# marvinpfoertner/linpde-gp

Hardware: AMD Instinct MI355X
Metric: condition+predict fp64 GFLOP/s (algorithmic), N=16384 Poisson-2D (higher is better)
Workload: dtype f64; 1 GPU; poisson2d_dirichlet_128x128; n_collocation=16384, n_other_observations=512, n_total=16896, m_predict=4096, multi_gpu=single GPU, rccl_ranks=0, device=(gfx950:sramecc+:xnack-), lazy_factorization=True, fused_factor_and_predict=True

## Files before the change

### linpde-gp_amd/csrc/api.hip

```cpp

#include <cstdarg>
#include <cstdlib>
#include <cstring>
#include <memory>

#include <rccl/rccl.h>

#include "lpgp_internal.h"

namespace lpgp {

static hipEvent_t get_event(lpgp_ctx* ctx) {
  if (!ctx->event_pool.empty()) {
    hipEvent_t e = ctx->event_pool.back();
    ctx->event_pool.pop_back();
    return e;
  }
  hipEvent_t e = nullptr;
  (void)hipEventCreate(&e);
  return e;
}

void prof_begin(lpgp_ctx* ctx, hipStream_t stream, int kernel, double flops, double bytes) {
  ctx->prof_open = 0;
// ... 255 lines not shown
  mat->cap = cap;
  mat->lr_cap = lr;
  mat->lc_cap = lc;
  mat->has_r = 0;
  return 0;
}

static void scatter_padded(const lpgp_mat* mat, const double* logical, double* padded) {
  std::memset(padded, 0, (size_t)mat->pn * sizeof(double));
  for (const auto& b : mat->blocks) std::memcpy(padded + b.poff, logical + b.off, (size_t)b.n * sizeof(double));
}
static void gather_padded(const lpgp_mat* mat, const double* padded, double* logical) {
  for (const auto& b : mat->blocks) std::memcpy(logical + b.off, padded + b.poff, (size_t)b.n * sizeof(double));
}

}

using namespace lpgp;

extern "C" {

const char* lpgp_last_error(void) { return lpgp::last_error(); }

int lpgp_init(int device, lpgp_ctx** out) {
  LPGP_CHECK(out != nullptr, "lpgp_init: null out");
  int ndev = 0;
  LPGP_HIP(hipGetDeviceCount(&ndev));
  LPGP_CHECK(ndev > 0, "lpgp_init: no HIP device visible (this library has no CPU fallback)");
  LPGP_CHECK(device >= 0 && device < ndev, "lpgp_init: device %d out of range (%d visible)", device, ndev);
  LPGP_HIP(hipSetDevice(device));
  lpgp_ctx* ctx = new lpgp_ctx();
  ctx->device = device;
  options_from_env(*ctx);
  hipDeviceProp_t prop;
  LPGP_HIP(hipGetDeviceProperties(&prop, device));
  ctx->cus = prop.multiProcessorCount;
  int lo = 0, hi = 0;
  LPGP_HIP(hipDeviceGetStreamPriorityRange(&lo, &hi));
  LPGP_HIP(hipStreamCreateWithPriority(&ctx->s_main, hipStreamNonBlocking, hi));
  auto masked_stream = [&](int nreserve, hipStream_t* out) {
    *out = nullptr;
    if (nreserve == 0 || nreserve >= ctx->cus) return;
    const int words = (ctx->cus + 31) / 32;
    std::vector<uint32_t> mask(words, 0u);
    for (int cu = 0; cu < ctx->cus; ++cu) mask[cu / 32] |= (1u << (cu % 32));
    for (int r = 0; r < nreserve; ++r) mask[r / 32] &= ~(1u << (r % 32));
    if (hipExtStreamCreateWithCUMask(out, (uint32_t)words, mask.data()) != hipSuccess) {
      (void)hipGetLastError();
      *out = nullptr;
    }
  };
  if (ctx->single_stream) {
    ctx->s_upd = ctx->s_upd_narrow = ctx->s_upd_all = ctx->s_outer = ctx->s_main;
  } else {
  masked_stream(ctx->reserve_cus, &ctx->s_upd);
  if (!ctx->s_upd) LPGP_HIP(hipStreamCreateWithPriority(&ctx->s_upd, hipStreamNonBlocking, lo));
  masked_stream(ctx->reserve_narrow, &ctx->s_upd_narrow);
  LPGP_HIP(hipStreamCreateWithPriority(&ctx->s_upd_all, hipStreamNonBlocking, lo));
  masked_stream(ctx->reserve_cus, &ctx->s_outer);
  if (!ctx->s_outer) LPGP_HIP(hipStreamCreateWithPriority(&ctx->s_outer, hipStreamNonBlocking, lo));
  }
  for (int i = 0; i < 2; ++i) {
    LPGP_HIP(hipEventCreateWithFlags(&ctx->ev_outer[i], hipEventDisableTiming));
    LPGP_HIP(hipEventCreateWithFlags(&ctx->ev_outer_fact[i], hipEventDisableTiming));
    LPGP_HIP(hipEventCreateWithFlags(&ctx->ev_outer_a1[i], hipEventDisableTiming));
  }
  for (int i = 0; i < 4; ++i) LPGP_HIP(hipEventCreateWithFlags(&ctx->ev_ride[i], hipEventDisableTiming));
  LPGP_HIP(hipEventCreateWithFlags(&ctx->ev_chain_pre, hipEventDisableTiming));
  LPGP_HIP(hipEventCreateWithFlags(&ctx->ev_chain_rows, hipEventDisableTiming));
  LPGP_HIP(hipEventCreateWithFlags(&ctx->ev_append[0], hipEventDisableTiming));
  LPGP_HIP(hipEventCreateWithFlags(&ctx->ev_append[1], hipEventDisableTiming));
  for (int i = 0; i < 2; ++i) {
    LPGP_HIP(hipEventCreateWithFlags(&ctx->ev_panel[i], hipEventDisableTiming));
    LPGP_HIP(hipEventCreateWithFlags(&ctx->ev_upd[i], hipEventDisableTiming));
  }
  for (auto& sl : ctx->desc_ring) {
    LPGP_HIP(hipHostMalloc(&sl.h, sizeof(DevDesc), hipHostMallocDefault));
    LPGP_HIP(hipMalloc(&sl.d, sizeof(DevDesc)));
    LPGP_HIP(hipEventCreateWithFlags(&sl.done, hipEventDisableTiming));
  }
  LPGP_HIP(hipMalloc(&ctx->d_info, sizeof(int)));
  LPGP_HIP(hipHostMalloc(&ctx->h_info_pinned, 64, hipHostMallocDefault));
  *out = ctx;
  return 0;
}

int lpgp_finalize(lpgp_ctx* ctx) {
  if (!ctx) return 0;
  (void)hipSetDevice(ctx->device);
  if (ctx->nccl_comm && ctx->world > 1 && sync_stream(ctx, ctx->s_main) != 0) {
  }
  (void)hipDeviceSynchronize();
  for (auto& p : ctx->pending) {
    (void)hipEventDestroy(p.e0);
    (void)hipEventDestroy(p.e1);
  }
  for (auto e : ctx->event_pool) (void)hipEventDestroy(e);
  for (int i = 0; i < 4; ++i) (void)hipEventDestroy(ctx->ev_ride[i]);
  (void)hipEventDestroy(ctx->ev_chain_pre);
  if (ctx->ev_chain_rows) (void)hipEventDestroy(ctx->ev_chain_rows);
  for (auto& e : ctx->ev_append) if (e) (void)hipEventDestroy(e);
  for (int i = 0; i < 2; ++i) {
    (void)hipEventDestroy(ctx->ev_panel[i]);
    (void)hipEventDestroy(ctx->ev_upd[i]);
    (void)hipEventDestroy(ctx->ev_outer[i]);
    (void)hipEventDestroy(ctx->ev_outer_fact[i]);
    (void)hipEventDestroy(ctx->ev_outer_a1[i]);
  }
  for (auto& sl : ctx->desc_ring) {
    (void)hipHostFree(sl.h);
    (void)hipFree(sl.d);
    (void)hipEventDestroy(sl.done);
  }
  (void)hipFree(ctx->d_info);
  if (ctx->d_chain_flags) (void)hipFree(ctx->d_chain_flags);
  (void)hipHostFree(ctx->h_info_pinned);
  if (ctx->h_stage) (void)hipHostFree(ctx->h_stage);
  for (auto& b : ctx->pts_pool) (void)hipFree(b.p);
  ctx->pts_pool.clear();
  for (auto& sl : ctx->pts_ring) {
    if (sl.h) (void)hipHostFree(sl.h);
    if (sl.done) (void)hipEventDestroy(sl.done);
  }
  if (ctx->h_stage_r) (void)hipHostFree(ctx->h_stage_r);
  if (ctx->ev_stage_r) (void)hipEventDestroy(ctx->ev_stage_r);
  if (ctx->d_tmp) (void)hipFree(ctx->d_tmp);
  for (size_t r = 0; r < ctx->ipc_peer.size(); ++r)
    if ((int)r != ctx->rank && ctx->ipc_peer[r]) (void)hipIpcCloseMemHandle(ctx->ipc_peer[r]);
  if (ctx->ipc_window) (void)hipFree(ctx->ipc_window);
  for (int i = 0; i < 2; ++i)
    if (ctx->ev_ipc[i]) (void)hipEventDestroy(ctx->ev_ipc[i]);
// ... 11 lines not shown
  for (auto& b : ctx->pool) (void)hipFree(b.p);
  ctx->pool.clear();
  if (!ctx->single_stream) {
    (void)hipStreamDestroy(ctx->s_upd);
    if (ctx->s_upd_narrow) (void)hipStreamDestroy(ctx->s_upd_narrow);
    (void)hipStreamDestroy(ctx->s_upd_all);
    if (ctx->s_outer) (void)hipStreamDestroy(ctx->s_outer);
  }
  (void)hipStreamDestroy(ctx->s_main);
  delete ctx;
  return 0;
}

int lpgp_device_info(lpgp_ctx* ctx, char* name, int len, int* cus, int64_t* hbm_bytes) {
  LPGP_DEVICE(ctx);
  hipDeviceProp_t prop;
  LPGP_HIP(hipGetDeviceProperties(&prop, ctx->device));
  if (name && len > 0) {
    std::snprintf(name, (size_t)len, "%s (%s)", prop.name, prop.gcnArchName);
  }
  if (cus) *cus = prop.multiProcessorCount;
  if (hbm_bytes) *hbm_bytes = (int64_t)prop.totalGlobalMem;
  return 0;
}

int lpgp_sync(lpgp_ctx* ctx) {
  LPGP_HIP(hipSetDevice(ctx->device));
  LPGP_HIP(hipDeviceSynchronize());
  return 0;
}

#define ROUTE(name) {"route_" #name, &lpgp_ctx::RouteCounts::name}
static const struct { const char* key; int64_t lpgp_ctx::RouteCounts::*count; } kRoutes[] = {
    ROUTE(ride_done), ROUTE(ride_aug), ROUTE(ride_b2b), ROUTE(ride), ROUTE(ride_vchain), ROUTE(ride_two), ROUTE(ride_outer),
    ROUTE(solve_two_level), ROUTE(solve_ahead), ROUTE(solve_tiles)};
#undef ROUTE
static const struct { const char* key; int64_t lpgp_ctx::*field; } kEvidence[] = {
    {"inverse_diag_panel", &lpgp_ctx::inverse_diag_panel}, {"evidence_h2d_bytes", &lpgp_ctx::evidence_h2d_bytes}, {"evidence_d2h_bytes", &lpgp_ctx::evidence_d2h_bytes}};

int lpgp_get_option(lpgp_ctx* ctx, const char* key, int64_t* value) {
  LPGP_CHECK(ctx && key && value, "lpgp_get_option: null argument");
  const int rc = option_get(*ctx, key, value);
  if (rc == 0) return 0;
  if (std::strcmp(key, "live_mats") == 0) {
    *value = ctx->live_mats;
    return 0;
  }
  for (const auto& r : kRoutes)
    if (std::strcmp(key, r.key) == 0) {
      *value = ctx->route.*r.count;
      return 0;
    }
  for (const auto& r : kEvidence)
    if (std::strcmp(key, r.key) == 0) {
      *value = ctx->*r.field;
      return 0;
    }
  return rc;
}

int lpgp_set_option(lpgp_ctx* ctx, const char* key, int64_t value) {
  LPGP_DEVICE(ctx);
  if (key && std::strcmp(key, kEvidence[0].key) == 0) {
    LPGP_CHECK(value >= TILE && value <= 4096 && value % TILE == 0, "inverse_diag_panel must be a multiple of %d in %d .. 4096", TILE, TILE);
    ctx->inverse_diag_panel = value;
    return 0;
  }
  return option_set(*ctx, key, value);
}

int lpgp_dist_unique_id(char* out128) {
  LPGP_CHECK(out128 != nullptr, "lpgp_dist_unique_id: null argument");
  static_assert(sizeof(ncclUniqueId) == 128, "ncclUniqueId size");
  ncclUniqueId id;
  ncclResult_t r = ncclGetUniqueId(&id);
  LPGP_CHECK(r == ncclSuccess, "ncclGetUniqueId: %s", ncclGetErrorString(r));
  std::memcpy(out128, &id, 128);
  return 0;
}

static void choose_grid(lpgp_ctx* ctx, int world) {
  if (ctx->grid_set && ctx->pr * ctx->pc == world) return;
  ctx->pr = world;
  ctx->pc = 1;
}

static int dist_fail(lpgp_ctx* ctx, int rc);

int lpgp_dist_set_grid(lpgp_ctx* ctx, int32_t pr, int32_t pc) {
  LPGP_CHECK(ctx && pr >= 1 && pc >= 1 && pr <= 8 && pc <= 8, "lpgp_dist_set_grid: bad grid %d x %d", pr, pc);
  if (ctx->distributed()) {
    LPGP_CHECK(pr * pc == ctx->world, "lpgp_dist_set_grid: grid %d x %d does not match %d ranks", pr, pc, ctx->world);
    LPGP_CHECK(ctx->live_mats == 0, "lpgp_dist_set_grid: %d matrices / right-hand sides of the current grid are still alive", ctx->live_mats);
  }
  ctx->pr = pr;
  ctx->pc = pc;
  ctx->grid_set = 1;
  return 0;
// ... 982 lines not shown
  const bool via_z = mean_host && var_host && !mat->has_w && mat->has_r;
  if (mean_host && !via_z) {
    LPGP_CHECK(mat->has_w, "lpgp_predict: representer weights not computed (call lpgp_solve_weights%s)",
               var_host ? " or lpgp_mat_set_residual" : "");
    LPGP_TRY(reduce_read_back(ctx, mat, K, mat->w, false, prior_mean_host, nullptr, mean_host, nullptr, nullptr));
  }
  if (var_host) {
    LPGP_CHECK(kxx_host != nullptr, "lpgp_predict: kxx_host required for the variance");
    double* zcol = K->v + (int64_t)K->m * K->ld;
    if (via_z)
      LPGP_HIP(hipMemcpyAsync(zcol, mat->r(), (size_t)mat->pn * sizeof(double), hipMemcpyDeviceToDevice, ctx->s_main));
    LPGP_TRY(solve_lower(ctx, mat, K->v, K->ld, K->m_pad));
    LPGP_TRY(reduce_read_back(ctx, mat, K, via_z ? zcol : nullptr, true, prior_mean_host, kxx_host, mean_host, var_host, nullptr));
  }
  return 0;
}

int lpgp_potrf_predict(lpgp_ctx* ctx, lpgp_mat* mat, lpgp_rhs* K, const double* prior_mean_host, const double* kxx_host,
                       double* mean_host, double* var_host) {
  LPGP_CHECK(ctx && mat && K && kxx_host && mean_host && var_host, "lpgp_potrf_predict: null argument");
  LPGP_DEVICE(ctx);
  LPGP_MAT_ALIVE(mat, "lpgp_potrf_predict");
  LPGP_CHECK(!ctx->distributed(), "lpgp_potrf_predict: single GPU only (a multi-GPU job factors collectively: lpgp_potrf, lpgp_predict)");
  LPGP_CHECK(mat->hidden.empty(), "lpgp_potrf_predict: a strict prefix of the blocks is in view");
  LPGP_CHECK(K->ld == mat->pn && mat->pn > 0, "lpgp_potrf_predict: right-hand side built for another matrix size");
  LPGP_CHECK(mat->has_r, "lpgp_potrf_predict: no residual resident (lpgp_mat_set_residual)");
  LPGP_TRY(ensure_tmp(ctx, 2 * K->m_pad));
  LPGP_TRY(ensure_stage(ctx, 2 * K->m_pad));
  LPGP_TRY(rhs_clear_unassembled(ctx, mat, K));
  double* zcol = K->v + (int64_t)K->m * K->ld;
  LPGP_HIP(hipMemcpyAsync(zcol, mat->r(), (size_t)mat->pn * sizeof(double), hipMemcpyDeviceToDevice, ctx->s_main));
  const bool fresh = mat->pn_fact < mat->pn;
  ctx->d_info_cur = mat->d_status;
  const int rc = potrf_predict_blocked(ctx, mat, mat->pn_fact / TILE, mat->pn / TILE, K->v, K->ld, K->m_pad);
  if (rc != 0) {
    if (fresh) mat->poisoned = 1;
    return rc;
  }
  if (fresh) {
    mat->pn_fact = mat->pn;
    mat->unchecked = 1;
    mat->has_w = 0;
  }
  mat->status_known = 0;
  int* const hinfo = ctx->h_info_pinned + 4;
  LPGP_TRY(reduce_read_back(ctx, mat, K, zcol, true, prior_mean_host, kxx_host, mean_host, var_host, hinfo));
  if (mat->unchecked) {
    mat->status_value = *hinfo;
    mat->status_known = 1;
  }
  return 0;
}

int lpgp_rhs_inner(lpgp_ctx* ctx, lpgp_rhs* A, lpgp_rhs* B, double* out_host) {
  LPGP_CHECK(ctx && A && B && out_host, "lpgp_rhs_inner: null argument");
  LPGP_DEVICE(ctx);
  LPGP_CHECK(A->ld == B->ld, "lpgp_rhs_inner: row mismatch");
  const int64_t ma = A->m_pad, mb = B->m_pad;
  std::vector<double> h((size_t)ma * mb);
  DevBuf dc;
  LPGP_TRY(DevBuf::raw(h.size() * sizeof(double), &dc));
  StreamDrain drain{ctx->s_main};
  GemmArgs g;
  g.A = A->v; g.B = B->v; g.C = dc.as(); g.lda = A->ld; g.ldb = B->ld; g.ldc = ma;
  g.mt = (int)(ma / TILE); g.nt = (int)(mb / TILE); g.k = (int)A->ld; g.alpha = 1.0; g.beta = 0.0;
  g.tri = 0;
  LPGP_TRY(launch_gemm(ctx, ctx->s_main, 1, 1, g, LPGP_K_GEMM));
// ... 295 lines not shown
```

### linpde-gp_amd/csrc/lpgp_internal.h

```cpp
#pragma once

#include <hip/hip_runtime.h>

#include <cstdint>
#include <cstdio>
#include <string>
#include <vector>

#include "lpgp.h"
#include "lpgp_desc.h"
#include "options.h"

namespace lpgp {

struct Cyc {
  int32_t P = 1, me = 0, nbt = 4;
};
__host__ __device__ inline int cyc_owner(const Cyc& c, int g) { return (g / c.nbt) % c.P; }
__host__ __device__ inline int cyc_before(const Cyc& c, int g) {
  const int B = g / c.nbt, rem = g - B * c.nbt;
  return ((B + c.P - 1 - c.me) / c.P) * c.nbt + ((B % c.P) == c.me ? rem : 0);
}
__host__ __device__ inline int cyc_l2g(const Cyc& c, int l) {
  const int lb = l / c.nbt;
// ... 25 lines not shown
  do {                            \
    int _rc = (expr);             \
    if (_rc != 0) return _rc;     \
  } while (0)
#define LPGP_TRY(expr) LPGP_TRY_RC(expr)

struct ProfSlot {
  double ms = 0.0;
  int64_t launches = 0;
  double flops = 0.0;
  double bytes = 0.0;
};

struct PendingEvent {
  hipEvent_t e0, e1;
  int kernel;
};

}

struct lpgp_ctx : lpgp::Options {
  int device = 0;
  int cus = 0;
  hipStream_t s_main = nullptr;
  hipStream_t s_upd = nullptr;
  hipStream_t s_upd_narrow = nullptr;
  hipStream_t s_upd_all = nullptr;
  hipStream_t s_outer = nullptr;
  hipEvent_t ev_outer[2] = {nullptr, nullptr};
  hipEvent_t ev_outer_fact[2] = {nullptr, nullptr};
  hipEvent_t ev_outer_a1[2] = {nullptr, nullptr};
  hipEvent_t ev_chain_pre = nullptr;
  hipEvent_t ev_ride[4] = {nullptr, nullptr, nullptr, nullptr};
  hipEvent_t ev_append[2] = {nullptr, nullptr};
  hipEvent_t ev_chain_rows = nullptr;
  int* d_chain_flags = nullptr;
  int64_t chain_launches = 0;
  int* chain_last_slot = nullptr;
  int chain_last_p0 = -1;
  struct RouteCounts {
    int64_t ride_done = 0;
    int64_t ride_aug = 0;
    int64_t ride_b2b = 0;
    int64_t ride = 0;
    int64_t ride_vchain = 0;
    int64_t ride_two = 0;
    int64_t ride_outer = 0;
    int64_t solve_two_level = 0;
    int64_t solve_ahead = 0;
    int64_t solve_tiles = 0;
  } route;
  hipEvent_t ev_panel[2] = {nullptr, nullptr};
  hipEvent_t ev_upd[2] = {nullptr, nullptr};
  int64_t inverse_diag_panel = 4096;
  int64_t evidence_h2d_bytes = 0, evidence_d2h_bytes = 0;
  int panel_lds_extra = 0;
  static constexpr int DESC_RING = 8;
  struct DescSlot { lpgp::DevDesc* h = nullptr; lpgp::DevDesc* d = nullptr; hipEvent_t done = nullptr; bool used = false; };
  DescSlot desc_ring[DESC_RING];
  int desc_next = 0;
  int* d_info = nullptr;
  int* d_info_cur = nullptr;
  int* h_info_pinned = nullptr;
  double* d_tmp = nullptr;
  int64_t tmp_cap = 0;
  double* h_stage = nullptr;
  double* h_stage_r = nullptr;
  int64_t stage_r_cap = 0;
  hipEvent_t ev_stage_r = nullptr;
  int64_t stage_cap = 0;
  struct PoolBuf { void* p; size_t bytes; };
  std::vector<PoolBuf> pool;
  std::vector<PoolBuf> pts_pool;
  static constexpr int PTS_SLOTS = 8;
  static constexpr size_t PTS_SLOT_BYTES = 64 << 10;
  struct PtsSlot { void* h = nullptr; hipEvent_t done = nullptr; bool used = false; };
  PtsSlot pts_ring[PTS_SLOTS];
  int pts_next = 0;
  int rank = 0, world = 1;
  int pr = 1, pc = 1;
  int grid_set = 0;
  int dist_broken = 0;
  int live_mats = 0;
  double comm_bytes_sent = 0.0, comm_bytes_recv = 0.0;
  hipStream_t s_comm = nullptr;
  hipEvent_t ev_comm[2] = {nullptr, nullptr};
  void* nccl_comm = nullptr;
  void* nccl_comm_bulk = nullptr;
// ... 196 lines not shown
  int32_t occ3 = 1;
  int32_t sshift = 3;
  int32_t dense = 0;
  int32_t ntiles = 0, chunk = 0, nbands = 0, band = 8;
  static constexpr int MAXB = 192;
  int32_t band_prefix[MAXB + 1];
  int32_t cyc = 0;
  Cyc rowc, colc;
  int32_t rt0 = 0, ct0 = 0, g0 = 0;
  unsigned long long* stamps = nullptr;
  unsigned long long* timeline = nullptr;
};
int launch_gemm(lpgp_ctx* ctx, hipStream_t stream, int ta, int tb, const GemmArgs& g, int prof_kernel);
int stair_enumerate_host(const GemmArgs& g, int32_t* out, int64_t cap);
int64_t gemm_valid_tiles(const GemmArgs& g);
int launch_trsv_tile(lpgp_ctx* ctx, hipStream_t stream, double* V, int64_t ldv, const double* linv, const double* L, int64_t ldl,
                     int nt, int prof_kernel);
int launch_trsm_tile(lpgp_ctx* ctx, hipStream_t stream, double* X, int64_t ldx, const double* linv, const double* L, int64_t ldl,
                     int mt, int prof_kernel);
int launch_trsv_panel(lpgp_ctx* ctx, hipStream_t stream, double* V, int64_t ldv, const double* linv, const double* L, int64_t ldl,
                      int nt_rows, int nt_cols, int prof_kernel);
int launch_trsv_panel_ahead(lpgp_ctx* ctx, hipStream_t stream, double* V, int64_t ldv, const double* linv, const double* L, const double* Lprev,
                            int64_t ldl, int nt_rows, int nt_cols, int prof_kernel);
int launch_trsm_panel(lpgp_ctx* ctx, hipStream_t stream, double* X, int64_t ldx, const double* linv, const double* L, int64_t ldl,
                      int nt_cols, int mt, int prof_kernel);

int launch_panel_chain(lpgp_ctx* ctx, hipStream_t stream, lpgp_mat* mat, int p0, int T, int* d_info, bool rows_here = true, bool ahead = false);
int launch_panel_chain_rows(lpgp_ctx* ctx, hipStream_t stream, lpgp_mat* mat, int p0, int T, int* d_info);
int launch_panel_chain_v(lpgp_ctx* ctx, hipStream_t stream, lpgp_mat* mat, int p0, double* V, int64_t ldv, int64_t cols, int* d_info);
int debug_tile_xcc(int32_t* out8, int reset);
int launch_potrf_tile(lpgp_ctx* ctx, hipStream_t stream, double* a, int64_t lda, double* linv,
                      int* d_info, int info_base);
int potrf_blocked(lpgp_ctx* ctx, lpgp_mat* mat, int64_t t_done, int64_t T, int32_t* info);
int potrf_predict_blocked(lpgp_ctx* ctx, lpgp_mat* mat, int64_t t_done, int64_t T, double* v, int64_t ldv, int64_t m_pad);
int potrf_dist(lpgp_ctx* ctx, lpgp_mat* mat, int64_t t_done, int64_t T, int32_t* info);
int trsm_lower_dist(lpgp_ctx* ctx, lpgp_mat* mat, int64_t T, double* v, int64_t ldv, int64_t m_pad);
int trsm_lower_t_dist(lpgp_ctx* ctx, lpgp_mat* mat, int64_t T, double* v, int64_t ldv, int64_t m_pad);
int factor_to_host_dist(lpgp_ctx* ctx, lpgp_mat* mat, double* out_padded );
int copy2d(hipStream_t st, double* dst, int64_t ldd, const double* src, int64_t lds, int64_t rows, int64_t cols);
int trsm_lower_blocked(lpgp_ctx* ctx, lpgp_mat* mat, int64_t T, double* v, int64_t ldv, int64_t m_pad);
int trsm_lower_t_blocked(lpgp_ctx* ctx, lpgp_mat* mat, int64_t T, double* v, int64_t ldv, int64_t m_pad);
int solve_vec(lpgp_ctx* ctx, lpgp_mat* mat, int64_t T, double* v, double* tmp, int* info);
int solve_vec_resident(lpgp_ctx* ctx, lpgp_mat* mat, int64_t T, double* v, double* tmp, int* info);
int solve_vec_fwd(lpgp_ctx* ctx, hipStream_t st, lpgp_mat* mat, int64_t T, double* b, double* x);
int solve_vec_fwd_resident(lpgp_ctx* ctx, lpgp_mat* mat, int64_t T, const double* b, double* x, int* info);
int mat_evidence(lpgp_ctx* ctx, lpgp_mat* mat, const double* r_host, double out_host[2]);
int mat_inverse_diag(lpgp_ctx* ctx, lpgp_mat* mat, double* out_host);
int mat_loo(lpgp_ctx* ctx, lpgp_mat* mat, const double* r_host, const double* y_host, double* mean_host, double* var_host, double* logp_host);
int mat_inverse_into(lpgp_ctx* ctx, lpgp_mat* mat, lpgp_mat* out);
int mat_evidence_grad(lpgp_ctx* ctx, lpgp_mat* mat, const lpgp_mat* ginv, const lpgp_mat* dG, const double* r_host, double out_host[2]);
int mat_evidence_grad_diag(lpgp_ctx* ctx, lpgp_mat* mat, const lpgp_mat* ginv, int32_t bi, const double* v_host, double scalar, const double* r_host,
                           double out_host[2]);
int factor_matmul(lpgp_ctx* ctx, lpgp_mat* mat, const double* Z_host, int64_t s, const double* shift_host, double* out_host);

int launch_assemble(lpgp_ctx* ctx, hipStream_t stream, const DevDesc& host_desc, const double* x0,
                    int64_t n0, int64_t n0_pad, const double* x1, int64_t n1, int64_t n1_pad,
                    double* out, int64_t ld, int64_t row_off, int64_t col_off, int lower_only,
                    const Layout2D& lay = Layout2D());
struct AsmJob {
  const double* x0; int64_t n0, n0_pad;
  const double* x1; int64_t n1, n1_pad;
  int64_t row_off, col_off;
  int lower_only;
};
int assemble_weighted(lpgp_ctx* ctx, hipStream_t stream, const lpgp_wpair* pairs, int npairs, const double* w0_host, int A0,
                      const double* w1_host, int A1, const lpgp_pts* X0, const lpgp_pts* X1, bool sym, double* out, int64_t ld,
                      int64_t row_off, int64_t col_off, const Layout2D& lay);
// ... 20 lines not shown
```

### linpde-gp_amd/csrc/potrf.hip

```cpp

#include <climits>
#include <cstdlib>

#include <algorithm>

#include "lpgp_internal.h"
#include "kernel_util.h"
#include "potrf_tile.h"

namespace lpgp {

__global__ __launch_bounds__(TILE_WAVES * 64) void potrf_tile_kernel(double* __restrict__ a, int64_t lda,
                                                          double* __restrict__ linv, int* __restrict__ info,
                                                          int info_base) {
  extern __shared__ __attribute__((aligned(16))) double sm[];
  potrf_tile_body(a, lda, linv, info, info_base, sm);
}

int debug_tile_xcc(int32_t* out8, int reset) {
  int h[8];
  LPGP_HIP(hipMemcpyFromSymbol(h, HIP_SYMBOL(g_tile_xcc_hist), sizeof(h)));
  for (int i = 0; i < 8; ++i) out8[i] = h[i];
  if (reset) {
    int z[8] = {0, 0, 0, 0, 0, 0, 0, 0};
// ... 6 lines not shown
                      int* d_info, int info_base) {
  const size_t shmem = (size_t)TILE_LDS_DOUBLES * sizeof(double);
  LPGP_TRY_RC(ensure_lds_attr(ctx, reinterpret_cast<const void*>(&potrf_tile_kernel), shmem));
  prof_begin(ctx, stream, LPGP_K_POTRF_TILE, (double)TILE * TILE * TILE / 3.0, 0.0);
  hipLaunchKernelGGL(potrf_tile_kernel, dim3(1), dim3(TILE_WAVES * 64), shmem, stream, a, lda, linv, d_info, info_base);
  prof_end(ctx, stream);
  LPGP_HIP(hipGetLastError());
  return 0;
}

static inline GemmArgs mk(const double* A, int64_t lda, const double* B, int64_t ldb, double* C,
                          int64_t ldc, int mt, int nt, int k, double alpha, double beta, int tri) {
  GemmArgs g;
  g.A = A; g.B = B; g.C = C; g.lda = lda; g.ldb = ldb; g.ldc = ldc;
  g.mt = mt; g.nt = nt; g.k = k; g.alpha = alpha; g.beta = beta;
  g.tri = tri;
  return g;
}

static inline int panel_trsm(lpgp_ctx* ctx, hipStream_t st, lpgp_mat* mat, int jt, double* X, int mt) {
  const int64_t ld = mat->cap;
  return launch_trsm_tile(ctx, st, X, ld, mat->linv + (int64_t)jt * TILE * TILE, mat->a + (int64_t)jt * TILE * (ld + 1), ld, mt,
                          LPGP_K_TRSM);
}

struct Ride {
  double* v = nullptr;
  int64_t ldv = 0;
  int mtl = 0;
  hipStream_t stream = nullptr;
  hipStream_t stream2 = nullptr;
  hipEvent_t ev[2] = {nullptr, nullptr};
  int it = 0;
  int gate_pct = 100;
  int outer_t = 0;
  int blk_q0 = 0;
  bool open = true;
  std::vector<std::pair<int, int>> held;
  int64_t chain_launches0 = 0;
};
static int ride_panel_now(lpgp_ctx* ctx, lpgp_mat* mat, int T, int p0, int p1, Ride* rd, bool sync_first, bool resident = false);

static int ride_panel(lpgp_ctx* ctx, lpgp_mat* mat, int T, int p0, int p1, Ride* rd, bool old_panel = false, bool resident = false) {
  if (!rd->open && old_panel && ctx->ride_old_ungated && rd->held.empty()) return ride_panel_now(ctx, mat, T, p0, p1, rd, true);
  if (!rd->open) {
    if ((int64_t)(T - p1) * 100 > (int64_t)rd->gate_pct * T && p1 < T) {
      rd->held.emplace_back(p0, p1);
      return 0;
    }
    rd->open = true;
    bool first = true;
    for (auto& h : rd->held) {
      LPGP_TRY(ride_panel_now(ctx, mat, T, h.first, h.second, rd, first));
      first = false;
    }
    const bool none_held = rd->held.empty();
    rd->held.clear();
    return ride_panel_now(ctx, mat, T, p0, p1, rd, true, resident && none_held);
  }
  return ride_panel_now(ctx, mat, T, p0, p1, rd, true, resident);
}

static int ride_panel_now(lpgp_ctx* ctx, lpgp_mat* mat, int T, int p0, int p1, Ride* rd, bool sync_first, bool resident) {
  const int64_t ld = mat->cap, tb = TILE;
  const double* a = mat->a;
  const bool two = rd->stream2 != nullptr && rd->stream2 != rd->stream && rd->mtl >= 8;
  const bool vchain = resident && sync_first && !two && ctx->fused_solve && p1 - p0 == 4 && ctx->ride_vchain_max_wgs > 0 &&
                      rd->mtl * 4 <= ctx->ride_vchain_max_wgs && ctx->chain_last_p0 == p0 && ctx->chain_launches - rd->chain_launches0 <= 24;
  if (vchain && rd->stream != ctx->s_main && ctx->ride_vchain_pre) LPGP_HIP(hipStreamWaitEvent(rd->stream, ctx->ev_chain_pre, 0));
  if (vchain) ++ctx->route.ride_vchain;
  if (two) ++ctx->route.ride_two;
  if (vchain)
    LPGP_TRY(launch_panel_chain_v(ctx, rd->stream, mat, p0, rd->v + (int64_t)p0 * tb, rd->ldv, (int64_t)rd->mtl * tb, ctx->d_info_cur));
  if (sync_first && (rd->stream != ctx->s_main || two)) {
    hipEvent_t ev = rd->ev[rd->it++ & 1];
    LPGP_HIP(hipEventRecord(ev, ctx->s_main));
    if (rd->stream != ctx->s_main) LPGP_HIP(hipStreamWaitEvent(rd->stream, ev, 0));
    if (two && rd->stream2 != ctx->s_main) LPGP_HIP(hipStreamWaitEvent(rd->stream2, ev, 0));
  }
  const int halves = two ? 2 : 1;
  for (int q0 = p0; q0 < p1; q0 += 4) {
    const int q1 = (q0 + 4 < p1) ? q0 + 4 : p1;
    int lim = T, outer_from = -1, outer_q0 = 0;
    if (rd->outer_t > 0) {
      const int E = rd->blk_q0 + rd->outer_t;
      lim = std::min(T, E + 3);
      if (q1 >= E || q1 >= T) {
        outer_from = lim; outer_q0 = rd->blk_q0;
        rd->blk_q0 = q1;
      }
    }
    for (int h = 0; h < halves; ++h) {
      hipStream_t sV = h == 0 ? rd->stream : rd->stream2;
      const int c0 = (h == 0) ? 0 : rd->mtl / 2, c1 = (two && h == 0) ? rd->mtl / 2 : rd->mtl;
      double* vh = rd->v + (int64_t)c0 * tb * rd->ldv;
      const int mtl = c1 - c0;
      double* Vq = vh + (int64_t)q0 * tb;
      if (vchain) {
      } else if (ctx->fused_solve) {
        LPGP_TRY(launch_trsv_panel(ctx, sV, Vq, rd->ldv, mat->linv + (int64_t)q0 * tb * tb, a + (int64_t)q0 * tb * (ld + 1), ld, q1 - q0, mtl,
                                   LPGP_K_PANEL));
      } else {
        for (int jt = q0; jt < q1; ++jt) {
          double* Vj = vh + (int64_t)jt * tb;
          LPGP_TRY(launch_trsv_tile(ctx, sV, Vj, rd->ldv, mat->linv + (int64_t)jt * tb * tb, a + (int64_t)jt * tb * (ld + 1), ld, mtl, LPGP_K_TRSM));
          if (jt + 1 < q1)
            LPGP_TRY(launch_gemm(ctx, sV, 0, 1,
                                 mk(a + (int64_t)(jt + 1) * tb + (int64_t)jt * tb * ld, ld, Vj, rd->ldv, vh + (int64_t)(jt + 1) * tb, rd->ldv,
                                    q1 - jt - 1, mtl, TILE, -1.0, 1.0, 0),
                                 LPGP_K_GEMM));
        }
      }
      if (q1 < lim) {
        GemmArgs g = mk(a + (int64_t)q1 * tb + (int64_t)q0 * tb * ld, ld, Vq, rd->ldv, vh + (int64_t)q1 * tb, rd->ldv, lim - q1, mtl,
                        (q1 - q0) * TILE, -1.0, 1.0, 0);
// ... 123 lines not shown
    } else {
      have_upd_event = 0;
    }
    p0 = p1;
  }
  if (la && last_upd) LPGP_HIP(hipStreamWaitEvent(sP, last_upd, 0));
  return 0;
}

static int potrf_blocked_impl(lpgp_ctx* ctx, lpgp_mat* mat, int64_t t_done64, int64_t T64, int32_t* info, Ride* ride, int TR = 0);
int potrf_blocked(lpgp_ctx* ctx, lpgp_mat* mat, int64_t t_done64, int64_t T64, int32_t* info) {
  return potrf_blocked_impl(ctx, mat, t_done64, T64, info, nullptr);
}

__global__ __launch_bounds__(256) void transpose_kernel(double* __restrict__ dst, int64_t ldd, const double* __restrict__ src, int64_t lds) {
  __shared__ double t[32][33];
  const int tx = threadIdx.x & 31, ty = threadIdx.x >> 5;
  const int64_t r0 = (int64_t)blockIdx.x * 32, c0 = (int64_t)blockIdx.y * 32;
#pragma unroll
  for (int k = 0; k < 4; ++k) t[ty + 8 * k][tx] = src[r0 + tx + (c0 + ty + 8 * k) * lds];
  __syncthreads();
#pragma unroll
  for (int k = 0; k < 4; ++k) dst[c0 + tx + (r0 + ty + 8 * k) * ldd] = t[tx][ty + 8 * k];
}
static int transpose(hipStream_t st, double* dst, int64_t ldd, const double* src, int64_t lds, int64_t rows, int64_t cols) {
  for (int64_t c0 = 0; c0 < cols; c0 += 32 * 65535) {
    const int64_t nc = std::min<int64_t>(cols - c0, 32 * 65535);
    hipLaunchKernelGGL(transpose_kernel, dim3((unsigned)(rows / 32), (unsigned)(nc / 32)), dim3(256), 0, st, dst + c0, ldd, src + c0 * lds, lds);
  }
  LPGP_HIP(hipGetLastError());
  return 0;
}

int potrf_predict_blocked(lpgp_ctx* ctx, lpgp_mat* mat, int64_t t_done, int64_t T, double* v, int64_t ldv, int64_t m_pad) {
  Ride rd;
  rd.v = v; rd.ldv = ldv; rd.mtl = (int)(m_pad / TILE);
  rd.chain_launches0 = ctx->chain_launches;
  hipStream_t cand[5] = {ctx->s_outer, ctx->s_upd_all, ctx->s_upd_narrow, ctx->s_main, ctx->s_upd};
  const int i1 = ctx->ride_stream & 7, i2 = (ctx->ride_stream >> 3) & 7;
  rd.stream = (i1 < 5 && cand[i1]) ? cand[i1] : ctx->s_main;
  rd.stream2 = (i2 < 5 && cand[i2]) ? cand[i2] : nullptr;
  if (ctx->single_stream) { rd.stream = ctx->s_main; rd.stream2 = nullptr; }
  rd.ev[0] = ctx->ev_ride[0]; rd.ev[1] = ctx->ev_ride[1];
  if (T <= ctx->ride_same_stream_max_tiles) { rd.stream = ctx->s_main; rd.stream2 = nullptr; }
  rd.gate_pct = ctx->ride_gate_pct >= 0 ? ctx->ride_gate_pct : (T <= 192 ? 65 : 100);
  rd.open = rd.gate_pct >= 100 || rd.stream == ctx->s_main;
  rd.outer_t = (ctx->ride_outer_rows >= 8 * TILE && T >= ctx->ride_outer_min_tiles && T >= 2 * (ctx->ride_outer_rows / TILE)) ? (int)(ctx->ride_outer_rows / TILE) : 0;
  LPGP_HIP(hipEventRecord(ctx->ev_ride[2], ctx->s_main));
  if (rd.stream != ctx->s_main) LPGP_HIP(hipStreamWaitEvent(rd.stream, ctx->ev_ride[2], 0));
  if (rd.stream2 && rd.stream2 != ctx->s_main) LPGP_HIP(hipStreamWaitEvent(rd.stream2, ctx->ev_ride[2], 0));
  if (t_done >= T) {
    ++ctx->route.ride_done;
    return trsm_lower_blocked(ctx, mat, T, v, ldv, m_pad);
  }
  if (ctx->ride_aug && (T + rd.mtl) * (int64_t)TILE <= mat->cap && !ctx->single_stream) {
    ++ctx->route.ride_aug;
    double* vt = mat->a + T * (int64_t)TILE;
    LPGP_TRY(transpose(ctx->s_main, vt, mat->cap, v, ldv, T * (int64_t)TILE, m_pad));
    LPGP_TRY(potrf_blocked_impl(ctx, mat, t_done, T, nullptr, nullptr, (int)T + rd.mtl));
    return transpose(ctx->s_main, v, ldv, vt, mat->cap, m_pad, T * (int64_t)TILE);
  }
  if (T >= ctx->ride_max_tiles) {
    ++ctx->route.ride_b2b;
    LPGP_TRY(potrf_blocked_impl(ctx, mat, t_done, T, nullptr, nullptr));
    return trsm_lower_blocked(ctx, mat, T, v, ldv, m_pad);
  }
  ++ctx->route.ride;
  LPGP_TRY(potrf_blocked_impl(ctx, mat, t_done, T, nullptr, &rd));
  if (rd.stream != ctx->s_main) {
    LPGP_HIP(hipEventRecord(ctx->ev_ride[2], rd.stream));
    LPGP_HIP(hipStreamWaitEvent(ctx->s_main, ctx->ev_ride[2], 0));
  }
  if (rd.stream2 && rd.stream2 != ctx->s_main && rd.stream2 != rd.stream) {
    LPGP_HIP(hipEventRecord(ctx->ev_ride[3], rd.stream2));
    LPGP_HIP(hipStreamWaitEvent(ctx->s_main, ctx->ev_ride[3], 0));
  }
  return 0;
}

static int potrf_blocked_impl(lpgp_ctx* ctx, lpgp_mat* mat, int64_t t_done64, int64_t T64, int32_t* info, Ride* ride, int TR) {
  const int T = (int)T64, t_done = (int)t_done64;
  if (TR < T) TR = T;
  const int64_t ld = mat->cap;
  double* a = mat->a;
  const int nbt = (int)(ctx->nb / TILE);
  const int64_t tb = TILE;
  hipStream_t sP = ctx->s_main, sU = ctx->s_upd;
  ctx->d_info_cur = info ? ctx->d_info : mat->d_status;
  if (info) LPGP_HIP(hipMemsetAsync(ctx->d_info, 0, sizeof(int), sP));

  hipEvent_t append_dep = nullptr;
  if (t_done > 0 && T > t_done) {
    const int mnew = TR - t_done;
    double* rows = a + (int64_t)t_done * tb;
    for (int p0 = 0; p0 < t_done; p0 += nbt) {
      const int p1 = (p0 + nbt < t_done) ? p0 + nbt : t_done;
      if (ctx->fused_solve && p1 - p0 <= 4) {
        LPGP_TRY(launch_trsm_panel(ctx, sP, rows + (int64_t)p0 * tb * ld, ld, mat->linv + (int64_t)p0 * tb * tb,
                                   a + (int64_t)p0 * tb * (ld + 1), ld, p1 - p0, mnew, LPGP_K_PANEL));
      } else
      for (int jt = p0; jt < p1; ++jt) {
// ... 457 lines not shown
```

### linpde-gp_amd/csrc/testhooks.hip

```cpp

#include <cstdlib>

#include "lpgp_internal.h"
#include "lpgp_test.h"

namespace lpgp {

typedef double v4f64 __attribute__((ext_vector_type(4)));

__global__ __launch_bounds__(256) void mfma_probe_kernel(double* out, int iters) {
  v4f64 acc[8];
  const double a = 1.0 + threadIdx.x * 1e-9, b = 1.0 - threadIdx.x * 1e-9;
#pragma unroll
  for (int i = 0; i < 8; ++i) acc[i] = (v4f64){0.0, 0.0, 0.0, 0.0};
  for (int it = 0; it < iters; ++it) {
#pragma unroll
    for (int i = 0; i < 8; ++i) acc[i] = __builtin_amdgcn_mfma_f64_16x16x4f64(a, b, acc[i], 0, 0, 0);
  }
  double s = 0.0;
#pragma unroll
  for (int i = 0; i < 8; ++i) s += acc[i][0] + acc[i][1] + acc[i][2] + acc[i][3];
  out[blockIdx.x * (int64_t)blockDim.x + threadIdx.x] = s;
}

// ... 181 lines not shown
  hipLaunchKernelGGL(write_probe_kernel, dim3(grid), dim3(256), 0, ctx->s_main, d, bytes / 16);
  LPGP_HIP(hipEventRecord(ev.e0, ctx->s_main));
  for (int r = 0; r < 5; ++r)
    hipLaunchKernelGGL(write_probe_kernel, dim3(grid), dim3(256), 0, ctx->s_main, d, bytes / 16);
  LPGP_HIP(hipEventRecord(ev.e1, ctx->s_main));
  LPGP_HIP(hipEventSynchronize(ev.e1));
  float ms = 0.f;
  LPGP_HIP(hipEventElapsedTime(&ms, ev.e0, ev.e1));
  if (gbps) *gbps = 5.0 * (double)bytes / (ms * 1e-3) / 1e9;
  return 0;
}

int lpgp_test_force_status(lpgp_ctx* ctx, lpgp_mat* mat, int32_t value) {
  LPGP_CHECK(ctx && mat, "lpgp_test_force_status: null argument");
  LPGP_DEVICE(ctx);
  LPGP_HIP(hipStreamSynchronize(ctx->s_main));
  LPGP_HIP(hipMemcpy(mat->d_status, &value, sizeof(int), hipMemcpyHostToDevice));
  mat->unchecked = 1;
  mat->status_known = 0;
  return 0;
}

int lpgp_test_mat_raw(lpgp_ctx* ctx, lpgp_mat* mat, int32_t set, double* host) {
  LPGP_CHECK(ctx && mat && host && mat->pn > 0, "lpgp_test_mat_raw: bad argument");
  LPGP_DEVICE(ctx);
  LPGP_CHECK(!ctx->distributed(), "lpgp_test_mat_raw: single GPU only");
  LPGP_HIP(hipStreamSynchronize(ctx->s_main));
  const size_t row = (size_t)mat->pn * sizeof(double), ld = (size_t)mat->lr_cap * sizeof(double);
  if (set) LPGP_HIP(hipMemcpy2D(mat->a, ld, host, row, row, (size_t)mat->pn, hipMemcpyHostToDevice));
  else LPGP_HIP(hipMemcpy2D(host, row, mat->a, ld, row, (size_t)mat->pn, hipMemcpyDeviceToHost));
  return 0;
}

}
```

Baseline: 55090 GFLOP/s.

## Ride the residual vector solve on a separate stream during fused factorization

Instead of padding the prediction RHS with an extra tile column for the residual vector, the residual is solved as a vector alongside each panel step, using dedicated matvec kernels on the narrow update stream. This drops one tile of columns from the ride TRSM work, from m+TILE down to m, and moves the triangular solve of the residual into small overlapped kernels. The cost is extra stream synchronisation and single-block solve kernels that run serially per panel step, which may contend for CUs.

Result: no change. 55540 GFLOP/s, median of 6 (+0.8%).

```diff
diff --git a/linpde-gp_amd/csrc/api.hip b/linpde-gp_amd/csrc/api.hip
--- a/linpde-gp_amd/csrc/api.hip
+++ b/linpde-gp_amd/csrc/api.hip
@@ -311,6 +311,7 @@
   lpgp_ctx* ctx = new lpgp_ctx();
   ctx->device = device;
   options_from_env(*ctx);
+  if (const char* e = std::getenv("LPGP_RIDE_VEC")) ctx->ride_vec = std::max<int64_t>(0, std::atoll(e));
   hipDeviceProp_t prop;
   LPGP_HIP(hipGetDeviceProperties(&prop, device));
   ctx->cus = prop.multiProcessorCount;
@@ -345,6 +346,7 @@
     LPGP_HIP(hipEventCreateWithFlags(&ctx->ev_outer_a1[i], hipEventDisableTiming));
   }
   for (int i = 0; i < 4; ++i) LPGP_HIP(hipEventCreateWithFlags(&ctx->ev_ride[i], hipEventDisableTiming));
+  LPGP_HIP(hipEventCreateWithFlags(&ctx->ev_ride_z, hipEventDisableTiming));
   LPGP_HIP(hipEventCreateWithFlags(&ctx->ev_chain_pre, hipEventDisableTiming));
   LPGP_HIP(hipEventCreateWithFlags(&ctx->ev_chain_rows, hipEventDisableTiming));
   LPGP_HIP(hipEventCreateWithFlags(&ctx->ev_append[0], hipEventDisableTiming));
@@ -376,6 +378,7 @@
   }
   for (auto e : ctx->event_pool) (void)hipEventDestroy(e);
   for (int i = 0; i < 4; ++i) (void)hipEventDestroy(ctx->ev_ride[i]);
+  (void)hipEventDestroy(ctx->ev_ride_z);
   (void)hipEventDestroy(ctx->ev_chain_pre);
   if (ctx->ev_chain_rows) (void)hipEventDestroy(ctx->ev_chain_rows);
   for (auto& e : ctx->ev_append) if (e) (void)hipEventDestroy(e);
@@ -453,7 +456,7 @@
 
 #define ROUTE(name) {"route_" #name, &lpgp_ctx::RouteCounts::name}
 static const struct { const char* key; int64_t lpgp_ctx::RouteCounts::*count; } kRoutes[] = {
-    ROUTE(ride_done), ROUTE(ride_aug), ROUTE(ride_b2b), ROUTE(ride), ROUTE(ride_vchain), ROUTE(ride_two), ROUTE(ride_outer),
+    ROUTE(ride_done), ROUTE(ride_aug), ROUTE(ride_b2b), ROUTE(ride), ROUTE(ride_vchain), ROUTE(ride_two), ROUTE(ride_outer), ROUTE(ride_held), ROUTE(ride_vec),
     ROUTE(solve_two_level), ROUTE(solve_ahead), ROUTE(solve_tiles)};
 #undef ROUTE
 static const struct { const char* key; int64_t lpgp_ctx::*field; } kEvidence[] = {
@@ -477,6 +480,10 @@
       *value = ctx->*r.field;
       return 0;
     }
+  if (std::strcmp(key, "ride_vec") == 0) {
+    *value = ctx->ride_vec;
+    return 0;
+  }
   return rc;
 }
 
@@ -485,6 +492,11 @@
   if (key && std::strcmp(key, kEvidence[0].key) == 0) {
     LPGP_CHECK(value >= TILE && value <= 4096 && value % TILE == 0, "inverse_diag_panel must be a multiple of %d in %d .. 4096", TILE, TILE);
     ctx->inverse_diag_panel = value;
+    return 0;
+  }
+  if (key && std::strcmp(key, "ride_vec") == 0) {
+    LPGP_CHECK(value >= 0, "ride_vec must be >= 0 (tile rows from which the residual rides as a vector; 0: never)");
+    ctx->ride_vec = value;
     return 0;
   }
   return option_set(*ctx, key, value);
@@ -1533,7 +1545,8 @@
   LPGP_HIP(hipMemcpyAsync(zcol, mat->r(), (size_t)mat->pn * sizeof(double), hipMemcpyDeviceToDevice, ctx->s_main));
   const bool fresh = mat->pn_fact < mat->pn;
   ctx->d_info_cur = mat->d_status;
-  const int rc = potrf_predict_blocked(ctx, mat, mat->pn_fact / TILE, mat->pn / TILE, K->v, K->ld, K->m_pad);
+  const bool zvec = ctx->ride_vec > 0 && mat->pn / TILE >= ctx->ride_vec && K->m % TILE == 0 && K->m_pad == K->m + TILE;
+  const int rc = potrf_predict_blocked(ctx, mat, mat->pn_fact / TILE, mat->pn / TILE, K->v, K->ld, zvec ? K->m : K->m_pad, zvec ? zcol : nullptr);
   if (rc != 0) {
     if (fresh) mat->poisoned = 1;
     return rc;
diff --git a/linpde-gp_amd/csrc/lpgp_internal.h b/linpde-gp_amd/csrc/lpgp_internal.h
--- a/linpde-gp_amd/csrc/lpgp_internal.h
+++ b/linpde-gp_amd/csrc/lpgp_internal.h
@@ -81,6 +81,7 @@
   hipEvent_t ev_outer_a1[2] = {nullptr, nullptr};
   hipEvent_t ev_chain_pre = nullptr;
   hipEvent_t ev_ride[4] = {nullptr, nullptr, nullptr, nullptr};
+  hipEvent_t ev_ride_z = nullptr;
   hipEvent_t ev_append[2] = {nullptr, nullptr};
   hipEvent_t ev_chain_rows = nullptr;
   int* d_chain_flags = nullptr;
@@ -95,6 +96,8 @@
     int64_t ride_vchain = 0;
     int64_t ride_two = 0;
     int64_t ride_outer = 0;
+    int64_t ride_held = 0;
+    int64_t ride_vec = 0;
     int64_t solve_two_level = 0;
     int64_t solve_ahead = 0;
     int64_t solve_tiles = 0;
@@ -103,6 +106,7 @@
   hipEvent_t ev_upd[2] = {nullptr, nullptr};
   int64_t inverse_diag_panel = 4096;
   int64_t evidence_h2d_bytes = 0, evidence_d2h_bytes = 0;
+  int64_t ride_vec = 128;
   int panel_lds_extra = 0;
   static constexpr int DESC_RING = 8;
   struct DescSlot { lpgp::DevDesc* h = nullptr; lpgp::DevDesc* d = nullptr; hipEvent_t done = nullptr; bool used = false; };
@@ -365,7 +369,10 @@
 int launch_potrf_tile(lpgp_ctx* ctx, hipStream_t stream, double* a, int64_t lda, double* linv,
                       int* d_info, int info_base);
 int potrf_blocked(lpgp_ctx* ctx, lpgp_mat* mat, int64_t t_done, int64_t T, int32_t* info);
-int potrf_predict_blocked(lpgp_ctx* ctx, lpgp_mat* mat, int64_t t_done, int64_t T, double* v, int64_t ldv, int64_t m_pad);
+int potrf_predict_blocked(lpgp_ctx* ctx, lpgp_mat* mat, int64_t t_done, int64_t T, double* v, int64_t ldv, int64_t m_pad, double* z);
+int launch_ride_vec_solve(lpgp_ctx* ctx, hipStream_t stream, double* z, const double* linv, const double* L, int64_t ldl, int nt_rows);
+int launch_ride_vec_update(lpgp_ctx* ctx, hipStream_t stream, double* zb, const double* Lb, int64_t ldl, const double* zp, int mt_rows,
+                           int nt_cols);
 int potrf_dist(lpgp_ctx* ctx, lpgp_mat* mat, int64_t t_done, int64_t T, int32_t* info);
 int trsm_lower_dist(lpgp_ctx* ctx, lpgp_mat* mat, int64_t T, double* v, int64_t ldv, int64_t m_pad);
 int trsm_lower_t_dist(lpgp_ctx* ctx, lpgp_mat* mat, int64_t T, double* v, int64_t ldv, int64_t m_pad);
diff --git a/linpde-gp_amd/csrc/potrf.hip b/linpde-gp_amd/csrc/potrf.hip
--- a/linpde-gp_amd/csrc/potrf.hip
+++ b/linpde-gp_amd/csrc/potrf.hip
@@ -62,6 +62,8 @@
   hipStream_t stream2 = nullptr;
   hipEvent_t ev[2] = {nullptr, nullptr};
   int it = 0;
+  double* z = nullptr;
+  hipStream_t zstream = nullptr;
   int gate_pct = 100;
   int outer_t = 0;
   int blk_q0 = 0;
@@ -76,6 +78,7 @@
   if (!rd->open) {
     if ((int64_t)(T - p1) * 100 > (int64_t)rd->gate_pct * T && p1 < T) {
       rd->held.emplace_back(p0, p1);
+      ++ctx->route.ride_held;
       return 0;
     }
     rd->open = true;
@@ -102,15 +105,23 @@
   if (two) ++ctx->route.ride_two;
   if (vchain)
     LPGP_TRY(launch_panel_chain_v(ctx, rd->stream, mat, p0, rd->v + (int64_t)p0 * tb, rd->ldv, (int64_t)rd->mtl * tb, ctx->d_info_cur));
-  if (sync_first && (rd->stream != ctx->s_main || two)) {
+  const bool zaside = rd->z && rd->zstream != ctx->s_main;
+  if (sync_first && (rd->stream != ctx->s_main || two || zaside)) {
     hipEvent_t ev = rd->ev[rd->it++ & 1];
     LPGP_HIP(hipEventRecord(ev, ctx->s_main));
     if (rd->stream != ctx->s_main) LPGP_HIP(hipStreamWaitEvent(rd->stream, ev, 0));
     if (two && rd->stream2 != ctx->s_main) LPGP_HIP(hipStreamWaitEvent(rd->stream2, ev, 0));
+    if (zaside) LPGP_HIP(hipStreamWaitEvent(rd->zstream, ev, 0));
   }
   const int halves = two ? 2 : 1;
   for (int q0 = p0; q0 < p1; q0 += 4) {
     const int q1 = (q0 + 4 < p1) ? q0 + 4 : p1;
+    if (rd->z) {
+      LPGP_TRY(launch_ride_vec_solve(ctx, rd->zstream, rd->z + (int64_t)q0 * tb, mat->linv + (int64_t)q0 * tb * tb, a + (int64_t)q0 * tb * (ld + 1), ld,
+                                     q1 - q0));
+      LPGP_TRY(launch_ride_vec_update(ctx, rd->zstream, rd->z + (int64_t)q1 * tb, a + (int64_t)q1 * tb + (int64_t)q0 * tb * ld, ld,
+                                      rd->z + (int64_t)q0 * tb, T - q1, q1 - q0));
+    }
     int lim = T, outer_from = -1, outer_q0 = 0;
     if (rd->outer_t > 0) {
       const int E = rd->blk_q0 + rd->outer_t;
@@ -300,8 +311,14 @@
   return 0;
 }
 
-int potrf_predict_blocked(lpgp_ctx* ctx, lpgp_mat* mat, int64_t t_done, int64_t T, double* v, int64_t ldv, int64_t m_pad) {
+int potrf_predict_blocked(lpgp_ctx* ctx, lpgp_mat* mat, int64_t t_done, int64_t T, double* v, int64_t ldv, int64_t m_pad, double* z) {
+  const int64_t m_all = m_pad + (z ? TILE : 0);
+  const bool done = t_done >= T;
+  const bool aug = !done && ctx->ride_aug && (T + m_all / TILE) * (int64_t)TILE <= mat->cap && !ctx->single_stream;
+  const bool b2b = !done && !aug && T >= ctx->ride_max_tiles;
+  if (done || aug || b2b || !ctx->s_upd_narrow) { m_pad = m_all; z = nullptr; }
   Ride rd;
+  rd.z = z; rd.zstream = ctx->s_upd_narrow;
   rd.v = v; rd.ldv = ldv; rd.mtl = (int)(m_pad / TILE);
   rd.chain_launches0 = ctx->chain_launches;
   hipStream_t cand[5] = {ctx->s_outer, ctx->s_upd_all, ctx->s_upd_narrow, ctx->s_main, ctx->s_upd};
@@ -317,24 +334,30 @@
   LPGP_HIP(hipEventRecord(ctx->ev_ride[2], ctx->s_main));
   if (rd.stream != ctx->s_main) LPGP_HIP(hipStreamWaitEvent(rd.stream, ctx->ev_ride[2], 0));
   if (rd.stream2 && rd.stream2 != ctx->s_main) LPGP_HIP(hipStreamWaitEvent(rd.stream2, ctx->ev_ride[2], 0));
-  if (t_done >= T) {
+  if (rd.z && rd.zstream != ctx->s_main) LPGP_HIP(hipStreamWaitEvent(rd.zstream, ctx->ev_ride[2], 0));
+  if (done) {
     ++ctx->route.ride_done;
     return trsm_lower_blocked(ctx, mat, T, v, ldv, m_pad);
   }
-  if (ctx->ride_aug && (T + rd.mtl) * (int64_t)TILE <= mat->cap && !ctx->single_stream) {
+  if (aug) {
     ++ctx->route.ride_aug;
     double* vt = mat->a + T * (int64_t)TILE;
     LPGP_TRY(transpose(ctx->s_main, vt, mat->cap, v, ldv, T * (int64_t)TILE, m_pad));
     LPGP_TRY(potrf_blocked_impl(ctx, mat, t_done, T, nullptr, nullptr, (int)T + rd.mtl));
     return transpose(ctx->s_main, v, ldv, vt, mat->cap, m_pad, T * (int64_t)TILE);
   }
-  if (T >= ctx->ride_max_tiles) {
+  if (b2b) {
     ++ctx->route.ride_b2b;
     LPGP_TRY(potrf_blocked_impl(ctx, mat, t_done, T, nullptr, nullptr));
     return trsm_lower_blocked(ctx, mat, T, v, ldv, m_pad);
   }
   ++ctx->route.ride;
+  if (rd.z) ++ctx->route.ride_vec;
   LPGP_TRY(potrf_blocked_impl(ctx, mat, t_done, T, nullptr, &rd));
+  if (rd.z && rd.zstream != ctx->s_main) {
+    LPGP_HIP(hipEventRecord(ctx->ev_ride_z, rd.zstream));
+    LPGP_HIP(hipStreamWaitEvent(ctx->s_main, ctx->ev_ride_z, 0));
+  }
   if (rd.stream != ctx->s_main) {
     LPGP_HIP(hipEventRecord(ctx->ev_ride[2], rd.stream));
     LPGP_HIP(hipStreamWaitEvent(ctx->s_main, ctx->ev_ride[2], 0));
diff --git a/linpde-gp_amd/csrc/ride_vec.hip b/linpde-gp_amd/csrc/ride_vec.hip
--- /dev/null
+++ b/linpde-gp_amd/csrc/ride_vec.hip
@@ -0,0 +1,104 @@
+
+#include "lpgp_internal.h"
+
+namespace lpgp {
+
+namespace {
+
+constexpr int RV_THREADS = 256;
+
+__device__ __forceinline__ double rv_tile_mv(const double* __restrict__ M, int64_t ldm, const double* x, double* part, int t) {
+  const int r = t & 127, h = t >> 7;
+  const double* Mp = M + r + (int64_t)(64 * h) * ldm;
+  double a0 = 0.0, a1 = 0.0;
+#pragma unroll 8
+  for (int c = 0; c < 64; c += 2) {
+    a0 = fma(Mp[(int64_t)c * ldm], x[64 * h + c], a0);
+    a1 = fma(Mp[(int64_t)(c + 1) * ldm], x[64 * h + c + 1], a1);
+  }
+  part[t] = a0 + a1;
+  __syncthreads();
+  const double v = t < TILE ? part[t] + part[t + 128] : 0.0;
+  __syncthreads();
+  return v;
+}
+
+}
+
+__global__ __launch_bounds__(RV_THREADS) void ride_vec_solve_kernel(double* __restrict__ z, const double* __restrict__ linv,
+                                                                    const double* __restrict__ L, int64_t ldl, int nt) {
+  __shared__ double zs[4 * TILE], s1[TILE], s2[TILE], part[RV_THREADS];
+  const int t = threadIdx.x;
+  for (int i = t; i < nt * TILE; i += RV_THREADS) zs[i] = z[i];
+  __syncthreads();
+  for (int k = 0; k < nt; ++k) {
+    const double* li = linv + (int64_t)k * TILE * TILE;
+    const double* Lkk = L + (int64_t)k * TILE * (ldl + 1);
+    double* b = zs + k * TILE;
+    const double x0 = rv_tile_mv(li, TILE, b, part, t);
+    if (t < TILE) s1[t] = x0;
+    __syncthreads();
+    const double lx = rv_tile_mv(Lkk, ldl, s1, part, t);
+    if (t < TILE) s2[t] = b[t] - lx;
+    __syncthreads();
+    const double dx = rv_tile_mv(li, TILE, s2, part, t);
+    if (t < TILE) b[t] = x0 + dx;
+    __syncthreads();
+    for (int s = k + 1; s < nt; ++s) {
+      const double u = rv_tile_mv(L + (int64_t)s * TILE + (int64_t)k * TILE * ldl, ldl, b, part, t);
+      if (t < TILE) zs[s * TILE + t] -= u;
+    }
+    __syncthreads();
+  }
+  for (int i = t; i < nt * TILE; i += RV_THREADS) z[i] = zs[i];
+}
+
+__global__ __launch_bounds__(RV_THREADS) void ride_vec_update_kernel(double* __restrict__ zb, const double* __restrict__ Lb, int64_t ldl,
+                                                                     const double* __restrict__ zp, int kc) {
+  __shared__ double zs[4 * TILE];
+  __shared__ double2 part[4][64];
+  const int t = threadIdx.x, lane = t & 63, w = t >> 6;
+  for (int i = t; i < kc; i += RV_THREADS) zs[i] = zp[i];
+  __syncthreads();
+  const int64_t row0 = (int64_t)blockIdx.x * TILE;
+  const double* Lp = Lb + row0 + 2 * lane;
+  double2 acc = make_double2(0.0, 0.0);
+  for (int c0 = 8 * w; c0 < kc; c0 += 32) {
+    double2 l[8];
+#pragma unroll
+    for (int j = 0; j < 8; ++j) l[j] = *reinterpret_cast<const double2*>(Lp + (int64_t)(c0 + j) * ldl);
+#pragma unroll
+    for (int j = 0; j < 8; ++j) {
+      const double x = zs[c0 + j];
+      acc.x = fma(l[j].x, x, acc.x);
+      acc.y = fma(l[j].y, x, acc.y);
+    }
+  }
+  part[w][lane] = acc;
+  __syncthreads();
+  if (t < TILE) {
+    const double* p = reinterpret_cast<const double*>(&part[0][0]);
+    zb[row0 + t] -= (p[t] + p[TILE + t]) + (p[2 * TILE + t] + p[3 * TILE + t]);
+  }
+}
+
+int launch_ride_vec_solve(lpgp_ctx* ctx, hipStream_t stream, double* z, const double* linv, const double* L, int64_t ldl, int nt_rows) {
+  LPGP_CHECK(nt_rows >= 1 && nt_rows <= 4, "ride_vec: a panel step has 1 .. 4 tile rows");
+  ProfScope prof(ctx, stream, LPGP_K_TRSM, (double)nt_rows * (nt_rows + 1) / 2 * TILE * TILE, 0.0);
+  hipLaunchKernelGGL(ride_vec_solve_kernel, dim3(1), dim3(RV_THREADS), 0, stream, z, linv, L, ldl, nt_rows);
+  LPGP_HIP(hipGetLastError());
+  return 0;
+}
+
+int launch_ride_vec_update(lpgp_ctx* ctx, hipStream_t stream, double* zb, const double* Lb, int64_t ldl, const double* zp, int mt_rows,
+                           int nt_cols) {
+  LPGP_CHECK(nt_cols >= 1 && nt_cols <= 4, "ride_vec: a panel step has 1 .. 4 tile columns");
+  if (mt_rows <= 0) return 0;
+  const double n = (double)mt_rows * TILE * nt_cols * TILE;
+  ProfScope prof(ctx, stream, LPGP_K_MATVEC, 2.0 * n, 8.0 * n);
+  hipLaunchKernelGGL(ride_vec_update_kernel, dim3((unsigned)mt_rows), dim3(RV_THREADS), 0, stream, zb, Lb, ldl, zp, nt_cols * TILE);
+  LPGP_HIP(hipGetLastError());
+  return 0;
+}
+
+}
diff --git a/linpde-gp_amd/csrc/testhooks.hip b/linpde-gp_amd/csrc/testhooks.hip
--- a/linpde-gp_amd/csrc/testhooks.hip
+++ b/linpde-gp_amd/csrc/testhooks.hip
@@ -237,4 +237,12 @@
   return 0;
 }
 
-}
+int lpgp_test_rhs_spare(lpgp_ctx* ctx, lpgp_rhs* rhs, double* host) {
+  LPGP_CHECK(ctx && rhs && host && rhs->m_pad > rhs->m, "lpgp_test_rhs_spare: bad argument");
+  LPGP_DEVICE(ctx);
+  LPGP_HIP(hipStreamSynchronize(ctx->s_main));
+  LPGP_HIP(hipMemcpy(host, rhs->v + rhs->m * rhs->ld, (size_t)rhs->ld * sizeof(double), hipMemcpyDeviceToHost));
+  return 0;
+}
+
+}
```
